# waabox/domain-mcp-server

Measured on AMD Instinct MI355X. Metric: classes indexed/sec, higher is better.
Workload: dtype n/a (CPU text indexing); 1 GPU; model=synthetic-java-spring-monorepo-2000-classes, global_batch=2000, parallelism=dp1 (one repo per rank), enrichment=none

## Files before the change

### native/srcscan/project.cpp

```cpp
#include <algorithm>
#include <chrono>
#include <dirent.h>
#include <string>
#include <unordered_map>
#include <unordered_set>

#include "srcscan.hpp"

namespace srcscan {

void go_project_files(const std::string& root, int threads, std::string& module, std::vector<FileRec>& files,
                      std::string* go_json);

namespace {

struct Entry {
    std::string name;
    bool is_dir;
};

std::vector<Entry> entries(const std::string& dir) {
    std::vector<std::pair<std::string, bool>> raw;
    std::vector<Entry> out;
    if (!list_dir(dir, raw)) return out;
// ... 46 lines not shown
    w.key("methods");
    w.begin_arr();
    for (auto& m : f.methods) {
        w.begin_obj();
        w.kv("name", m.name);
        w.kv_int("line", m.line);
        w.kv_opt("httpMethod", m.has_http_method ? &m.http_method : nullptr);
        w.kv_opt("httpPath", m.has_http_path ? &m.http_path : nullptr);
        w.str_array("exceptions", m.exceptions);
        w.end_obj();
    }
    w.end_arr();
    w.end_obj();
}

void scan_java(const std::string& root, const ScanOptions& opt, ScanResult& res) {
    std::vector<FileRec>& files = res.files;
    const std::string src_root = "src/main/java";
    std::string abs_src = join_path(root, src_root);
    if (!dir_exists(abs_src)) return;
    std::vector<std::string> rels;
    auto t = std::chrono::steady_clock::now();
    walk(abs_src, "", [](const std::string& n) { return ends_with(n, ".java"); },
         [](const std::string&) { return false; }, rels);
    res.walk_us = us_since(t);
    t = std::chrono::steady_clock::now();
    files.resize(rels.size());
    std::vector<std::string> sources(rels.size());
    parallel_for(rels.size(), opt.threads, [&](size_t k) {
        FileRec& f = files[k];
        f.rel_path = src_root + "/" + rels[k];
        f.abs_path = join_path(root, f.rel_path);
        f.identifier = dotted(strip_ext(rels[k], ".java"));
        std::string src;
        if (!read_file(f.abs_path, src)) return;
        analyze_java(src, f);
    });
    for (auto& f : files) if (!f.parsed) ++res.skipped;
    res.analyze_us = us_since(t);
    t = std::chrono::steady_clock::now();
    std::unordered_set<std::string> known;
    known.reserve(files.size() * 2);
    for (auto& f : files) known.insert(f.identifier);
    parallel_for(files.size(), opt.threads, [&](size_t k) {
        FileRec& f = files[k];
        std::unordered_set<std::string> seen;
        std::unordered_map<std::string, std::string> import_map;
        for (auto& imp : f.imports) {
            if (imp.is_asterisk) continue;
            std::string fq = imp.imported;
            if (imp.is_static) {
                size_t d = fq.rfind('.');
// ... 267 lines not shown
```

### native/srcscan/pymodule.cpp

```cpp
#include <pybind11/pybind11.h>
#include <pybind11/stl.h>
#include <sys/random.h>

#include <cctype>
#include <chrono>
#include <cstring>
#include <deque>
#include <memory>
#include <thread>
#include <unordered_map>
#include <vector>

#include "bulkwriter.hpp"
#include "gitobj.hpp"
#include "graphjson.hpp"
#include "srcscan.hpp"
#include "wire.hpp"

namespace py = pybind11;

namespace {

dbw::Batch to_batch(const std::string& sql, py::handle rows) {
    dbw::Batch b;
    b.sql = sql;
    PyObject* seq = PySequence_Fast(rows.ptr(), "rows must be a sequence");
    if (!seq) throw py::error_already_set();
    py::object keep = py::reinterpret_steal<py::object>(seq);
    const Py_ssize_t n = PySequence_Fast_GET_SIZE(seq);
    if (n == 0) return b;
    PyObject** items = PySequence_Fast_ITEMS(seq);
    PyObject* first = items[0];
    if (!PyTuple_Check(first)) throw py::type_error("rows must be tuples");
    b.ncols = static_cast<int>(PyTuple_GET_SIZE(first));
    b.values.resize(static_cast<size_t>(n) * b.ncols);
    for (Py_ssize_t r = 0; r < n; ++r) {
// ... 14 lines not shown
            } else if (PyBool_Check(o) || PyLong_Check(o)) {
                v.kind = dbw::Value::Int;
                v.i = PyLong_AsLongLong(o);
                if (v.i == -1 && PyErr_Occurred()) throw py::error_already_set();
            } else if (PyFloat_Check(o)) {
                v.kind = dbw::Value::Real;
                v.d = PyFloat_AS_DOUBLE(o);
            } else {
                throw py::type_error("unsupported column value type");
            }
        }
    }
    return b;
}

srcscan::ScanResult scan_mounted(py::list files, const std::string& language, int threads,
                                 const std::string& framework, bool go_doc = true) {
    const auto t = std::chrono::steady_clock::now();
    std::vector<py::object> hold;
    hold.reserve(files.size());
    std::vector<std::pair<std::string, std::string_view>> tree;
    tree.reserve(files.size());
    for (auto item : files) {
        auto tup = item.cast<py::tuple>();
        if (tup.size() != 2) throw py::type_error("files: (path, bytes) pairs expected");
        PyObject* content = tup[1].ptr();
        char* data = nullptr;
        Py_ssize_t n = 0;
        if (!PyBytes_Check(content) || PyBytes_AsStringAndSize(content, &data, &n) < 0)
            throw py::type_error("files: content must be bytes");
        tree.emplace_back(tup[0].cast<std::string>(), std::string_view(data, static_cast<size_t>(n)));
        hold.push_back(std::move(tup));
    }
    py::gil_scoped_release release;
    std::string root = srcscan::vfs_mount_views(tree);
    const long long mount_us =
        std::chrono::duration_cast<std::chrono::microseconds>(std::chrono::steady_clock::now() - t).count();
    srcscan::ScanOptions opt;
    opt.language = language;
    opt.threads = threads;
    opt.framework = framework;
    opt.go_doc = go_doc;
    try {
        srcscan::ScanResult r = srcscan::scan_project(root, opt);
        r.mount_us = mount_us;
        srcscan::vfs_unmount(root);
        return r;
    } catch (...) {
        srcscan::vfs_unmount(root);
        throw;
    }
}

py::str pystr(const std::string& s) {
    PyObject* o = PyUnicode_DecodeUTF8(s.data(), static_cast<Py_ssize_t>(s.size()), "replace");
    if (!o) throw py::error_already_set();
    return py::reinterpret_steal<py::str>(o);
}

void json_str_list_ascii(PyObject* seq, std::string& out) {
    static const char* hex = "0123456789abcdef";
    out.push_back('[');
    const Py_ssize_t n = PySequence_Fast_GET_SIZE(seq);
    PyObject** items = PySequence_Fast_ITEMS(seq);
    for (Py_ssize_t i = 0; i < n; ++i) {
        if (i) out.append(", ");
// ... 22 lines not shown
                        u4(c);
                    } else if (c >= 0x10000) {
                        const unsigned v = c - 0x10000;
                        u4(0xd800 | (v >> 10));
                        u4(0xdc00 | (v & 0x3ff));
                    } else {
                        out.push_back((char)c);
                    }
            }
        }
        out.push_back('"');
    }
    out.push_back(']');
}

struct RowBuilder {
    dbw::Batch b;
    explicit RowBuilder(const std::string& sql, int ncols) {
        b.sql = sql;
        b.ncols = ncols;
    }
    void null() { b.values.emplace_back(); }
    void text(const char* p, Py_ssize_t n) {
        dbw::Value v;
        v.kind = dbw::Value::Text;
        v.p = p;
        v.n = static_cast<int32_t>(n);
        b.values.push_back(v);
    }
    void str(PyObject* o) {
        if (o == Py_None) return null();
        Py_ssize_t n = 0;
        const char* p = PyUnicode_AsUTF8AndSize(o, &n);
        if (!p) throw py::error_already_set();
        text(p, n);
    }
    void owned(std::string&& s) {
        b.owned.push_back(std::move(s));
        text(b.owned.back().data(), (Py_ssize_t)b.owned.back().size());
    }
    void integer_or_null(PyObject* o) {
        if (o == Py_None) return null();
        dbw::Value v;
        v.kind = dbw::Value::Int;
        v.i = PyLong_AsLongLong(o);
        if (v.i == -1 && PyErr_Occurred()) throw py::error_already_set();
        b.values.push_back(v);
    }
    void integer(long long i) {
        dbw::Value v;
        v.kind = dbw::Value::Int;
        v.i = i;
        b.values.push_back(v);
    }
    bool empty() const { return b.values.empty(); }
};

PyObject* getattr_borrowed(PyObject* o, const char* name, std::vector<py::object>& hold) {
    PyObject* a = PyObject_GetAttrString(o, name);
    if (!a) throw py::error_already_set();
    hold.emplace_back(py::reinterpret_steal<py::object>(a));
    return a;
}

struct StrCache {
    std::unordered_map<std::string_view, PyObject*> map;
    std::deque<std::string> owned;
    ~StrCache() {
        for (auto& kv : map) Py_DECREF(kv.second);
    }
// ... 100 lines not shown
        PyTuple_SET_ITEM(rec, 0, fresh(f.rel_path));
        PyTuple_SET_ITEM(rec, 1, fresh(f.identifier));
        PyTuple_SET_ITEM(rec, 2, shared.get(f.class_type));
        PyTuple_SET_ITEM(rec, 3, PyBool_FromLong(f.entry_point));
        PyTuple_SET_ITEM(rec, 4, shared.get(f.package_name));
        PyTuple_SET_ITEM(rec, 5, shared_list(f.deps));
        PyTuple_SET_ITEM(rec, 6, params);
        PyTuple_SET_ITEM(rec, 7, methods);
        PyList_SET_ITEM(files.ptr(), k, rec);
    }
    d["files"] = files;
    d["go"] = r.go_json.empty() ? py::object(py::none()) : py::object(pystr(r.go_json));
    return d;
}

struct Uuid7Gen {
    unsigned long long ms = 0, hi = 0, lo = 0;
    Uuid7Gen() {
        unsigned char seed[10];
        if (getrandom(seed, sizeof(seed), 0) != (ssize_t)sizeof(seed)) throw std::runtime_error("getrandom failed");
        ms = (unsigned long long)std::chrono::duration_cast<std::chrono::milliseconds>(
                 std::chrono::system_clock::now().time_since_epoch())
                 .count();
        hi = ((unsigned long long)(seed[0] & 0x07) << 8) | seed[1];
        for (int j = 2; j < 10; ++j) lo = (lo << 8) | seed[j];
        lo &= 0x1FFFFFFFFFFFFFFFull;
    }
    void next(char* s) {
        static const char* hex = "0123456789abcdef";
        unsigned char b[16];
        for (int j = 0; j < 6; ++j) b[j] = (unsigned char)(ms >> (8 * (5 - j)));
        b[6] = (unsigned char)(0x70 | ((hi >> 8) & 0x0F));
        b[7] = (unsigned char)(hi & 0xFF);
        b[8] = (unsigned char)(0x80 | ((lo >> 56) & 0x3F));
        for (int j = 9; j < 16; ++j) b[j] = (unsigned char)(lo >> (8 * (15 - j)));
        if (++lo >> 62) {
            lo = 0;
            ++hi;
        }
        int k = 0;
        for (int j = 0; j < 16; ++j) {
            if (j == 4 || j == 6 || j == 8 || j == 10) s[k++] = '-';
            s[k++] = hex[b[j] >> 4];
            s[k++] = hex[b[j] & 15];
        }
    }
};

void json_ascii_list(const std::vector<std::string>& v, std::string& out) {
    static const char* hex = "0123456789abcdef";
    auto u4 = [&](unsigned c) {
        out += "\\u";
        for (int sh = 12; sh >= 0; sh -= 4) out += hex[(c >> sh) & 15];
    };
    out = "[";
    for (size_t i = 0; i < v.size(); ++i) {
        if (i) out += ", ";
        out += '"';
        const std::string& s = v[i];
        for (size_t k = 0; k < s.size();) {
            unsigned char c = (unsigned char)s[k];
            unsigned cp = c;
            size_t len = 1;
            if (c >= 0xF0 && k + 3 < s.size() + 0) { cp = ((c & 7u) << 18) | ((s[k + 1] & 63u) << 12) | ((s[k + 2] & 63u) << 6) | (s[k + 3] & 63u); len = 4; }
            else if (c >= 0xE0 && k + 2 < s.size()) { cp = ((c & 15u) << 12) | ((s[k + 1] & 63u) << 6) | (s[k + 2] & 63u); len = 3; }
            else if (c >= 0xC0 && k + 1 < s.size()) { cp = ((c & 31u) << 6) | (s[k + 1] & 63u); len = 2; }
            k += len;
            if (cp == '"') out += "\\\"";
            else if (cp == '\\') out += "\\\\";
            else if (cp == '\n') out += "\\n";
            else if (cp == '\r') out += "\\r";
            else if (cp == '\t') out += "\\t";
            else if (cp == '\b') out += "\\b";
            else if (cp == '\f') out += "\\f";
            else if (cp < 0x20 || (cp >= 0x7f && cp < 0x10000)) u4(cp);
            else if (cp >= 0x10000) {
                cp -= 0x10000;
                u4(0xD800 + (cp >> 10));
                u4(0xDC00 + (cp & 0x3FF));
            } else out += (char)cp;
        }
        out += '"';
    }
    out += "]";
}

struct StaticRowsSpec {
    dbw::BulkWriter* writer = nullptr;
    std::string pid, now, commit, cls_sql, meth_sql;
    bool commit_null = false;
};

struct StaticRowsKeep {
    std::shared_ptr<const srcscan::ScanResult> r;
    StaticRowsSpec spec;
    std::string ids;
    std::vector<size_t> first;
    std::deque<std::string> strings;
};

const std::string& normalize_class_type(const std::string& t) {
    static const std::string kTypes[] = {"CONTROLLER", "SERVICE", "REPOSITORY", "ENTITY", "DTO",
                                         "CONFIGURATION", "LISTENER", "UTILITY", "EXCEPTION", "OTHER"};
    for (const std::string& k : kTypes) {
        if (k.size() != t.size()) continue;
        bool eq = true;
        for (size_t i = 0; i < t.size() && eq; ++i) eq = std::toupper((unsigned char)t[i]) == k[i];
        if (eq) return k;
    }
    return kTypes[9];
}

void emit_static_rows(const std::shared_ptr<StaticRowsKeep>& keep) {
    const srcscan::ScanResult& r = *keep->r;
    const StaticRowsSpec& spec = keep->spec;
    std::unordered_map<std::string_view, size_t> last;
    last.reserve(r.files.size() * 2);
    size_t n_ids = 0;
    for (size_t k = 0; k < r.files.size(); ++k) last[r.files[k].identifier] = k;
    for (size_t k = 0; k < r.files.size(); ++k)
        if (last[r.files[k].identifier] == k) n_ids += 1 + r.files[k].methods.size();
    keep->ids.resize(36 * n_ids);
    keep->first.assign(r.files.size(), std::string::npos);
    Uuid7Gen gen;
    size_t at = 0;
    const int chunk = 256;
    RowBuilder cls(spec.cls_sql, 10), meth(spec.meth_sql, 10);
    int pending = 0;
    auto flush = [&]() {
        cls.b.keep = keep;
        meth.b.keep = keep;
        if (!cls.empty()) spec.writer->put(std::move(cls.b));
        if (!meth.empty()) spec.writer->put(std::move(meth.b));
        cls = RowBuilder(spec.cls_sql, 10);
        meth = RowBuilder(spec.meth_sql, 10);
        pending = 0;
    };
    auto sv = [](RowBuilder& b, const std::string& s) { b.text(s.data(), (Py_ssize_t)s.size()); };
    for (size_t k = 0; k < r.files.size(); ++k) {
        const srcscan::FileRec& f = r.files[k];
        if (last[f.identifier] != k) continue;
        if (pending == chunk) flush();
        ++pending;
        keep->first[k] = at;
        const char* cid = &keep->ids[at];
        gen.next(&keep->ids[at]);
        at += 36;
        const std::string& ident = f.identifier;
        const size_t dot = ident.rfind('.');
        cls.text(cid, 36);
        sv(cls, spec.pid);
        sv(cls, ident);
        if (dot != std::string::npos) cls.text(ident.data() + dot + 1, (Py_ssize_t)(ident.size() - dot - 1));
        else sv(cls, ident);
        if (dot != std::string::npos) cls.text(ident.data(), (Py_ssize_t)dot); else cls.null();
        sv(cls, normalize_class_type(f.class_type));
        cls.null();
        sv(cls, f.rel_path);
        sv(cls, spec.now);
        if (spec.commit_null) cls.null(); else sv(cls, spec.commit);
        for (const srcscan::MethodRec& m : f.methods) {
            gen.next(&keep->ids[at]);
            meth.text(&keep->ids[at], 36);
            at += 36;
            meth.text(cid, 36);
            sv(meth, m.name);
            meth.null();
            meth.text("[]", 2);
            if (m.exceptions.empty()) {
                meth.text("[]", 2);
            } else {
                keep->strings.emplace_back();
                json_ascii_list(m.exceptions, keep->strings.back());
                sv(meth, keep->strings.back());
            }
            if (m.has_http_method) sv(meth, m.http_method); else meth.null();
            if (m.has_http_path) sv(meth, m.http_path); else meth.null();
            meth.integer(m.line);
            sv(meth, spec.now);
        }
    }
    flush();
}

py::tuple phase1_rows(dbw::BulkWriter& writer, py::list order, py::dict units, py::object ids, py::str pid,
                      py::str now, py::handle commit_hash, const std::string& cls_sql, const std::string& meth_sql,
                      const std::string& param_sql, py::handle method_info_cls, int chunk, py::object graph_targets,
                      py::object pre_ids) {
    if (!PyType_Check(method_info_cls.ptr()) ||
        !PyType_IsSubtype((PyTypeObject*)method_info_cls.ptr(), &PyTuple_Type))
        throw py::type_error("method_info_cls must be a tuple subclass");
    auto* mi_type = (PyTypeObject*)method_info_cls.ptr();
    const bool given = !ids.is_none();
    if (given && !PyList_Check(ids.ptr())) throw py::type_error("ids must be a list or None");
    const bool pre = !pre_ids.is_none();
    if (pre && (given || !PyDict_Check(pre_ids.ptr()))) throw py::type_error("pre_ids must be a dict (and ids None)");
    const Py_ssize_t n_ids = given ? PyList_GET_SIZE(ids.ptr()) : 0;
    Py_ssize_t next_id = 0;
    py::list generated;
// ... 253 lines not shown
            if (!lst) {
                if (PyErr_Occurred()) throw py::error_already_set();
                if (PyDict_SetItem(gper, mname, lks.ptr()) < 0) throw py::error_already_set();
            } else if (PyList_SetSlice(lst, PY_SSIZE_T_MAX, PY_SSIZE_T_MAX, lks.ptr()) < 0) {
                throw py::error_already_set();
            }
        }
    }
    if (!par.empty()) writer.put(std::move(par.b));
    return py::make_tuple(n_cls, n_meth, n_par, class_ids, class_types, method_infos, methods_by_ident, links,
                          generated);
}

}

py::dict objects_and_rows(std::shared_ptr<const srcscan::ScanResult> shared, py::handle method_cls, py::object rows) {
    std::shared_ptr<StaticRowsKeep> keep;
    std::thread emitter;
    std::atomic<long long> emit_us{0};
    if (!rows.is_none() && shared->language != "go") {
        py::tuple rt = rows.cast<py::tuple>();
        if (rt.size() != 6) throw py::value_error("rows must have 6 items");
        keep = std::make_shared<StaticRowsKeep>();
        keep->r = shared;
        StaticRowsSpec& spec = keep->spec;
        spec.writer = &rt[0].cast<dbw::BulkWriter&>();
        spec.pid = rt[1].cast<std::string>();
        spec.now = rt[2].cast<std::string>();
        spec.commit_null = rt[3].is_none();
        if (!spec.commit_null) spec.commit = rt[3].cast<std::string>();
        spec.cls_sql = rt[4].cast<std::string>();
        spec.meth_sql = rt[5].cast<std::string>();
        emitter = std::thread([keep, &emit_us] {
            const auto t = std::chrono::steady_clock::now();
            emit_static_rows(keep);
            emit_us = std::chrono::duration_cast<std::chrono::microseconds>(
                          std::chrono::steady_clock::now() - t).count();
        });
    }
    py::dict d;
    try {
        const auto t = std::chrono::steady_clock::now();
        d = scan_result_objects(*shared, method_cls);
        py::dict(d["stats"])["phaseUs"].cast<py::dict>()["objects"] =
            std::chrono::duration_cast<std::chrono::microseconds>(std::chrono::steady_clock::now() - t)
                .count();
    } catch (...) {
        if (emitter.joinable()) {
            py::gil_scoped_release release;
            emitter.join();
        }
        throw;
    }
    if (emitter.joinable()) {
        {
            py::gil_scoped_release release;
            emitter.join();
        }
        py::dict(d["stats"])["phaseUs"].cast<py::dict>()["rows"] = emit_us.load();
        py::dict row_ids;
        for (size_t k = 0; k < shared->files.size(); ++k) {
            const size_t at = keep->first[k];
            if (at == std::string::npos) continue;
            const size_t nm = shared->files[k].methods.size();
            py::list mids(nm);
            for (size_t j = 0; j < nm; ++j) mids[j] = py::str(&keep->ids[at + 36 * (j + 1)], 36);
            row_ids[pystr(shared->files[k].identifier)] = py::make_tuple(py::str(&keep->ids[at], 36), mids);
        }
        d["rowIds"] = row_ids;
    }
    keep.reset();
    std::thread([](std::shared_ptr<const srcscan::ScanResult>) {}, std::move(shared)).detach();
    return d;
}

PYBIND11_MODULE(_srcscan, m) {
    m.doc() = "Native Java / TypeScript / Go source front-ends for dmcp";
    m.def(
        "scan_project",
        [](const std::string& root, const std::string& language, int threads, const std::string& framework) {
            std::string out;
            {
                py::gil_scoped_release release;
                srcscan::ScanOptions opt;
                opt.language = language;
                opt.threads = threads;
// ... 23 lines not shown
                try {
                    out = srcscan::scan_project_json(root, opt);
                } catch (...) {
                    srcscan::vfs_unmount(root);
                    throw;
                }
                srcscan::vfs_unmount(root);
            }
            return py::bytes(out);
        },
        py::arg("files"), py::arg("language") = "auto", py::arg("threads") = 0, py::arg("framework") = "");
    m.def(
        "scan_sources_objects",
        [](py::list files, const std::string& language, int threads, const std::string& framework,
           py::handle method_cls, py::object rows, bool go_doc) {
            auto r = std::make_unique<srcscan::ScanResult>(scan_mounted(files, language, threads, framework,
                                                                        go_doc));
            return objects_and_rows(std::shared_ptr<const srcscan::ScanResult>(std::move(r)), method_cls, rows);
        },
        py::arg("files"), py::arg("language"), py::arg("threads"), py::arg("framework"), py::arg("method_cls"),
        py::arg("rows") = py::none(), py::arg("go_doc") = true,
        "scan_sources as Python objects (files as tuples, methods as method_cls) -- no JSON round trip; "
        "with rows, the class / method rows are written first (ids in 'rowIds'); go_doc=False: no "
        "go-analyzer package document (Go)");
    m.def(
        "result_objects",
        [](py::bytes blob, py::handle method_cls, py::object rows) {
            auto r = std::make_unique<srcscan::ScanResult>();
            std::string err;
            bool ok;
            {
                char* data = nullptr;
                Py_ssize_t n = 0;
                if (PyBytes_AsStringAndSize(blob.ptr(), &data, &n) < 0) throw py::error_already_set();
                py::gil_scoped_release release;
                ok = srcscan::decode_result(std::string_view(data, static_cast<size_t>(n)), *r, err);
            }
            if (!ok) throw py::value_error("scan result: " + err);
            return objects_and_rows(std::shared_ptr<const srcscan::ScanResult>(std::move(r)), method_cls, rows);
        },
        py::arg("blob"), py::arg("method_cls"), py::arg("rows") = py::none(),
        "the binary ScanResult of `srcscan serve` as scan_sources_objects returns it (untrusted bytes: every "
        "length checked)");
    m.def(
        "encode_scan",
        [](py::list files, const std::string& language, int threads, const std::string& framework, bool go_doc) {
            srcscan::ScanResult r = scan_mounted(files, language, threads, framework, go_doc);
            std::string out;
            {
                py::gil_scoped_release release;
                out = srcscan::encode_result(r, true);
            }
            return py::bytes(out);
        },
// ... 198 lines not shown
        .def_property_readonly("rows_written", &dbw::BulkWriter::rows_written)
        .def("timings", [](const dbw::BulkWriter& w) {
            py::dict d;
            d["setup_ms"] = w.setup_ms();
            d["rows_ms"] = w.rows_ms();
            d["commit_ms"] = w.commit_ms();
            d["idle_ms"] = w.idle_ms();
            d["free_ms"] = w.free_ms();
            d["open_ms"] = w.open_ms();
            d["t_start_s"] = w.t_start();
            d["t_setup_s"] = w.t_setup();
            d["t_commit_s"] = w.t_commit();
            d["t_end_s"] = w.t_end();
            return d;
        });
    m.attr("ABI_VERSION") = 6;
}
```

### native/srcscan/srcscan.hpp

```cpp
#pragma once

#include <string>
#include <vector>

#include "common.hpp"

namespace srcscan {

struct MethodRec {
    std::string name;
    int line = 0;
    bool has_http_method = false, has_http_path = false;
    std::string http_method, http_path;
    std::vector<std::string> exceptions;
    std::vector<std::string> param_types;
    bool is_ctor = false;
    bool params_eligible = true;
};

struct ImportRec {
    std::string imported;
    std::string local;
    std::string source;
    bool is_static = false;
// ... 23 lines not shown
    std::string name = "unknown";
    std::string source_root = "src";
    std::vector<std::pair<std::string, std::string>> features;
};
FrameworkInfo detect_framework(std::string_view package_json);

struct GoProject;
std::string analyze_go_project_json(const std::string& root, int threads);

struct ScanOptions {
    std::string language = "auto";
    int threads = 0;
    std::string framework;
    size_t max_file_bytes = 5u * 1024u * 1024u;
    bool go_doc = true;
};

struct ScanResult {
    std::string language;
    std::string source_root = ".";
    bool has_framework = false;
    FrameworkInfo framework;
    std::string module;
    std::string go_json;
    std::vector<FileRec> files;
    int skipped = 0;
    long long elapsed_us = 0;
    long long walk_us = 0, analyze_us = 0, resolve_us = 0, mount_us = 0;
};

// ... 15 lines not shown
```

Measured before the change: 51510 classes/s.

## Stream parsed Java files to the static row emitter during the scan

Adds a PrefixSink that hands contiguous ranges of finished files to a callback while the parallel Java analysis is still running. Static row emission moves into a separate staticrows module so it can feed those ranges from a dedicated thread, overlapping row building and database writes with parsing. The aim is to hide the serial post-scan emit phase behind the scan. In exchange it adds a mutex on every file completion, needs extra bookkeeping for duplicate identifiers, and makes error propagation more involved.

```diff
diff --git a/native/srcscan/project.cpp b/native/srcscan/project.cpp
--- a/native/srcscan/project.cpp
+++ b/native/srcscan/project.cpp
@@ -1,6 +1,8 @@
 #include <algorithm>
 #include <chrono>
 #include <dirent.h>
+#include <exception>
+#include <mutex>
 #include <string>
 #include <unordered_map>
 #include <unordered_set>
@@ -84,6 +86,58 @@
     w.end_obj();
 }
 
+class PrefixSink {
+public:
+    PrefixSink(const std::vector<FileRec>& files, const ScanOptions& opt)
+        : files_(files), sink_(opt.file_sink), chunk_(std::max<size_t>(1, opt.sink_chunk)) {
+        if (sink_) done_.assign(files.size(), 0);
+    }
+
+    void done(size_t k) {
+        if (!sink_) return;
+        std::unique_lock<std::mutex> lk(mu_);
+        done_[k] = 1;
+        while (prefix_ < done_.size() && done_[prefix_]) ++prefix_;
+        deliver(lk, chunk_);
+    }
+
+    void finish() {
+        if (!sink_) return;
+        std::unique_lock<std::mutex> lk(mu_);
+        deliver(lk, 1);
+        if (error_) std::rethrow_exception(error_);
+    }
+
+private:
+    void deliver(std::unique_lock<std::mutex>& lk, size_t at_least) {
+        if (delivering_) return;
+        delivering_ = true;
+        while (!error_ && prefix_ - sent_ >= at_least) {
+            const size_t first = sent_, last = prefix_;
+            sent_ = last;
+            lk.unlock();
+            std::exception_ptr err;
+            try {
+                sink_(files_, first, last);
+            } catch (...) {
+                err = std::current_exception();
+            }
+            lk.lock();
+            if (err) error_ = err;
+        }
+        delivering_ = false;
+    }
+
+    const std::vector<FileRec>& files_;
+    const std::function<void(const std::vector<FileRec>&, size_t, size_t)>& sink_;
+    const size_t chunk_;
+    std::mutex mu_;
+    std::vector<char> done_;
+    size_t prefix_ = 0, sent_ = 0;
+    bool delivering_ = false;
+    std::exception_ptr error_;
+};
+
 void scan_java(const std::string& root, const ScanOptions& opt, ScanResult& res) {
     std::vector<FileRec>& files = res.files;
     const std::string src_root = "src/main/java";
@@ -96,16 +150,20 @@
     res.walk_us = us_since(t);
     t = std::chrono::steady_clock::now();
     files.resize(rels.size());
-    std::vector<std::string> sources(rels.size());
     parallel_for(rels.size(), opt.threads, [&](size_t k) {
         FileRec& f = files[k];
         f.rel_path = src_root + "/" + rels[k];
         f.abs_path = join_path(root, f.rel_path);
         f.identifier = dotted(strip_ext(rels[k], ".java"));
+    });
+    PrefixSink sink(files, opt);
+    parallel_for(rels.size(), opt.threads, [&](size_t k) {
+        FileRec& f = files[k];
         std::string src;
-        if (!read_file(f.abs_path, src)) return;
-        analyze_java(src, f);
+        if (read_file(f.abs_path, src)) analyze_java(src, f);
+        sink.done(k);
     });
+    sink.finish();
     for (auto& f : files) if (!f.parsed) ++res.skipped;
     res.analyze_us = us_since(t);
     t = std::chrono::steady_clock::now();
diff --git a/native/srcscan/pymodule.cpp b/native/srcscan/pymodule.cpp
--- a/native/srcscan/pymodule.cpp
+++ b/native/srcscan/pymodule.cpp
@@ -15,11 +15,18 @@
 #include "gitobj.hpp"
 #include "graphjson.hpp"
 #include "srcscan.hpp"
+#include "staticrows.hpp"
 #include "wire.hpp"
 
 namespace py = pybind11;
 
 namespace {
+
+using staticrows::StaticRowsEmitter;
+using staticrows::StaticRowsKeep;
+using staticrows::StaticRowsSpec;
+using staticrows::stream_rows_enabled;
+using staticrows::Uuid7Gen;
 
 dbw::Batch to_batch(const std::string& sql, py::handle rows) {
     dbw::Batch b;
@@ -64,8 +71,10 @@
     return b;
 }
 
-srcscan::ScanResult scan_mounted(py::list files, const std::string& language, int threads,
-                                 const std::string& framework, bool go_doc = true) {
+void scan_mounted_into(py::list files, const std::string& language, int threads, const std::string& framework,
+                       bool go_doc, srcscan::ScanResult& r,
+                       std::function<void(const std::vector<srcscan::FileRec>&, size_t, size_t)> sink = nullptr,
+                       const std::function<void()>& after_scan = nullptr) {
     const auto t = std::chrono::steady_clock::now();
     std::vector<py::object> hold;
     hold.reserve(files.size());
@@ -91,15 +100,23 @@
     opt.threads = threads;
     opt.framework = framework;
     opt.go_doc = go_doc;
+    opt.file_sink = std::move(sink);
     try {
-        srcscan::ScanResult r = srcscan::scan_project(root, opt);
+        srcscan::scan_project_into(root, opt, r);
         r.mount_us = mount_us;
-        srcscan::vfs_unmount(root);
-        return r;
+        if (after_scan) after_scan();
     } catch (...) {
         srcscan::vfs_unmount(root);
         throw;
     }
+    srcscan::vfs_unmount(root);
+}
+
+srcscan::ScanResult scan_mounted(py::list files, const std::string& language, int threads,
+                                 const std::string& framework, bool go_doc = true) {
+    srcscan::ScanResult r;
+    scan_mounted_into(files, language, threads, framework, go_doc, r);
+    return r;
 }
 
 py::str pystr(const std::string& s) {
@@ -152,30 +169,14 @@
     out.push_back(']');
 }
 
-struct RowBuilder {
-    dbw::Batch b;
-    explicit RowBuilder(const std::string& sql, int ncols) {
-        b.sql = sql;
-        b.ncols = ncols;
-    }
-    void null() { b.values.emplace_back(); }
-    void text(const char* p, Py_ssize_t n) {
-        dbw::Value v;
-        v.kind = dbw::Value::Text;
-        v.p = p;
-        v.n = static_cast<int32_t>(n);
-        b.values.push_back(v);
-    }
+struct RowBuilder : staticrows::TextRows {
+    using staticrows::TextRows::TextRows;
     void str(PyObject* o) {
         if (o == Py_None) return null();
         Py_ssize_t n = 0;
         const char* p = PyUnicode_AsUTF8AndSize(o, &n);
         if (!p) throw py::error_already_set();
-        text(p, n);
-    }
-    void owned(std::string&& s) {
-        b.owned.push_back(std::move(s));
-        text(b.owned.back().data(), (Py_ssize_t)b.owned.back().size());
+        text(p, static_cast<size_t>(n));
     }
     void integer_or_null(PyObject* o) {
         if (o == Py_None) return null();
@@ -185,13 +186,6 @@
         if (v.i == -1 && PyErr_Occurred()) throw py::error_already_set();
         b.values.push_back(v);
     }
-    void integer(long long i) {
-        dbw::Value v;
-        v.kind = dbw::Value::Int;
-        v.i = i;
-        b.values.push_back(v);
-    }
-    bool empty() const { return b.values.empty(); }
 };
 
 PyObject* getattr_borrowed(PyObject* o, const char* name, std::vector<py::object>& hold) {
@@ -322,175 +316,6 @@
     return d;
 }
 
-struct Uuid7Gen {
-    unsigned long long ms = 0, hi = 0, lo = 0;
-    Uuid7Gen() {
-        unsigned char seed[10];
-        if (getrandom(seed, sizeof(seed), 0) != (ssize_t)sizeof(seed)) throw std::runtime_error("getrandom failed");
-        ms = (unsigned long long)std::chrono::duration_cast<std::chrono::milliseconds>(
-                 std::chrono::system_clock::now().time_since_epoch())
-                 .count();
-        hi = ((unsigned long long)(seed[0] & 0x07) << 8) | seed[1];
-        for (int j = 2; j < 10; ++j) lo = (lo << 8) | seed[j];
-        lo &= 0x1FFFFFFFFFFFFFFFull;
-    }
-    void next(char* s) {
-        static const char* hex = "0123456789abcdef";
-        unsigned char b[16];
-        for (int j = 0; j < 6; ++j) b[j] = (unsigned char)(ms >> (8 * (5 - j)));
-        b[6] = (unsigned char)(0x70 | ((hi >> 8) & 0x0F));
-        b[7] = (unsigned char)(hi & 0xFF);
-        b[8] = (unsigned char)(0x80 | ((lo >> 56) & 0x3F));
-        for (int j = 9; j < 16; ++j) b[j] = (unsigned char)(lo >> (8 * (15 - j)));
-        if (++lo >> 62) {
-            lo = 0;
-            ++hi;
-        }
-        int k = 0;
-        for (int j = 0; j < 16; ++j) {
-            if (j == 4 || j == 6 || j == 8 || j == 10) s[k++] = '-';
-            s[k++] = hex[b[j] >> 4];
-            s[k++] = hex[b[j] & 15];
-        }
-    }
-};
-
-void json_ascii_list(const std::vector<std::string>& v, std::string& out) {
-    static const char* hex = "0123456789abcdef";
-    auto u4 = [&](unsigned c) {
-        out += "\\u";
-        for (int sh = 12; sh >= 0; sh -= 4) out += hex[(c >> sh) & 15];
-    };
-    out = "[";
-    for (size_t i = 0; i < v.size(); ++i) {
-        if (i) out += ", ";
-        out += '"';
-        const std::string& s = v[i];
-        for (size_t k = 0; k < s.size();) {
-            unsigned char c = (unsigned char)s[k];
-            unsigned cp = c;
-            size_t len = 1;
-            if (c >= 0xF0 && k + 3 < s.size() + 0) { cp = ((c & 7u) << 18) | ((s[k + 1] & 63u) << 12) | ((s[k + 2] & 63u) << 6) | (s[k + 3] & 63u); len = 4; }
-            else if (c >= 0xE0 && k + 2 < s.size()) { cp = ((c & 15u) << 12) | ((s[k + 1] & 63u) << 6) | (s[k + 2] & 63u); len = 3; }
-            else if (c >= 0xC0 && k + 1 < s.size()) { cp = ((c & 31u) << 6) | (s[k + 1] & 63u); len = 2; }
-            k += len;
-            if (cp == '"') out += "\\\"";
-            else if (cp == '\\') out += "\\\\";
-            else if (cp == '\n') out += "\\n";
-            else if (cp == '\r') out += "\\r";
-            else if (cp == '\t') out += "\\t";
-            else if (cp == '\b') out += "\\b";
-            else if (cp == '\f') out += "\\f";
-            else if (cp < 0x20 || (cp >= 0x7f && cp < 0x10000)) u4(cp);
-            else if (cp >= 0x10000) {
-                cp -= 0x10000;
-                u4(0xD800 + (cp >> 10));
-                u4(0xDC00 + (cp & 0x3FF));
-            } else out += (char)cp;
-        }
-        out += '"';
-    }
-    out += "]";
-}
-
-struct StaticRowsSpec {
-    dbw::BulkWriter* writer = nullptr;
-    std::string pid, now, commit, cls_sql, meth_sql;
-    bool commit_null = false;
-};
-
-struct StaticRowsKeep {
-    std::shared_ptr<const srcscan::ScanResult> r;
-    StaticRowsSpec spec;
-    std::string ids;
-    std::vector<size_t> first;
-    std::deque<std::string> strings;
-};
-
-const std::string& normalize_class_type(const std::string& t) {
-    static const std::string kTypes[] = {"CONTROLLER", "SERVICE", "REPOSITORY", "ENTITY", "DTO",
-                                         "CONFIGURATION", "LISTENER", "UTILITY", "EXCEPTION", "OTHER"};
-    for (const std::string& k : kTypes) {
-        if (k.size() != t.size()) continue;
-        bool eq = true;
-        for (size_t i = 0; i < t.size() && eq; ++i) eq = std::toupper((unsigned char)t[i]) == k[i];
-        if (eq) return k;
-    }
-    return kTypes[9];
-}
-
-void emit_static_rows(const std::shared_ptr<StaticRowsKeep>& keep) {
-    const srcscan::ScanResult& r = *keep->r;
-    const StaticRowsSpec& spec = keep->spec;
-    std::unordered_map<std::string_view, size_t> last;
-    last.reserve(r.files.size() * 2);
-    size_t n_ids = 0;
-    for (size_t k = 0; k < r.files.size(); ++k) last[r.files[k].identifier] = k;
-    for (size_t k = 0; k < r.files.size(); ++k)
-        if (last[r.files[k].identifier] == k) n_ids += 1 + r.files[k].methods.size();
-    keep->ids.resize(36 * n_ids);
-    keep->first.assign(r.files.size(), std::string::npos);
-    Uuid7Gen gen;
-    size_t at = 0;
-    const int chunk = 256;
-    RowBuilder cls(spec.cls_sql, 10), meth(spec.meth_sql, 10);
-    int pending = 0;
-    auto flush = [&]() {
-        cls.b.keep = keep;
-        meth.b.keep = keep;
-        if (!cls.empty()) spec.writer->put(std::move(cls.b));
-        if (!meth.empty()) spec.writer->put(std::move(meth.b));
-        cls = RowBuilder(spec.cls_sql, 10);
-        meth = RowBuilder(spec.meth_sql, 10);
-        pending = 0;
-    };
-    auto sv = [](RowBuilder& b, const std::string& s) { b.text(s.data(), (Py_ssize_t)s.size()); };
-    for (size_t k = 0; k < r.files.size(); ++k) {
-        const srcscan::FileRec& f = r.files[k];
-        if (last[f.identifier] != k) continue;
-        if (pending == chunk) flush();
-        ++pending;
-        keep->first[k] = at;
-        const char* cid = &keep->ids[at];
-        gen.next(&keep->ids[at]);
-        at += 36;
-        const std::string& ident = f.identifier;
-        const size_t dot = ident.rfind('.');
-        cls.text(cid, 36);
-        sv(cls, spec.pid);
-        sv(cls, ident);
-        if (dot != std::string::npos) cls.text(ident.data() + dot + 1, (Py_ssize_t)(ident.size() - dot - 1));
-        else sv(cls, ident);
-        if (dot != std::string::npos) cls.text(ident.data(), (Py_ssize_t)dot); else cls.null();
-        sv(cls, normalize_class_type(f.class_type));
-        cls.null();
-        sv(cls, f.rel_path);
-        sv(cls, spec.now);
-        if (spec.commit_null) cls.null(); else sv(cls, spec.commit);
-        for (const srcscan::MethodRec& m : f.methods) {
-            gen.next(&keep->ids[at]);
-            meth.text(&keep->ids[at], 36);
-            at += 36;
-            meth.text(cid, 36);
-            sv(meth, m.name);
-            meth.null();
-            meth.text("[]", 2);
-            if (m.exceptions.empty()) {
-                meth.text("[]", 2);
-            } else {
-                keep->strings.emplace_back();
-                json_ascii_list(m.exceptions, keep->strings.back());
-                sv(meth, keep->strings.back());
-            }
-            if (m.has_http_method) sv(meth, m.http_method); else meth.null();
-            if (m.has_http_path) sv(meth, m.http_path); else meth.null();
-            meth.integer(m.line);
-            sv(meth, spec.now);
-        }
-    }
-    flush();
-}
-
 py::tuple phase1_rows(dbw::BulkWriter& writer, py::list order, py::dict units, py::object ids, py::str pid,
                       py::str now, py::handle commit_hash, const std::string& cls_sql, const std::string& meth_sql,
                       const std::string& param_sql, py::handle method_info_cls, int chunk, py::object graph_targets,
@@ -774,28 +599,36 @@
 
 }
 
-py::dict objects_and_rows(std::shared_ptr<const srcscan::ScanResult> shared, py::handle method_cls, py::object rows) {
-    std::shared_ptr<StaticRowsKeep> keep;
+std::unique_ptr<StaticRowsEmitter> rows_emitter(py::object rows, std::shared_ptr<const srcscan::ScanResult> shared) {
+    if (rows.is_none()) return nullptr;
+    py::tuple rt = rows.cast<py::tuple>();
+    if (rt.size() != 6) throw py::value_error("rows must have 6 items");
+    auto keep = std::make_shared<StaticRowsKeep>();
+    keep->r = std::move(shared);
+    StaticRowsSpec& spec = keep->spec;
+    spec.writer = &rt[0].cast<dbw::BulkWriter&>();
+    spec.pid = rt[1].cast<std::string>();
+    spec.now = rt[2].cast<std::string>();
+    spec.commit_null = rt[3].is_none();
+    if (!spec.commit_null) spec.commit = rt[3].cast<std::string>();
+    spec.cls_sql = rt[4].cast<std::string>();
+    spec.meth_sql = rt[5].cast<std::string>();
+    return std::make_unique<StaticRowsEmitter>(std::move(keep));
+}
+
+py::dict objects_and_rows(std::shared_ptr<const srcscan::ScanResult> shared, py::handle method_cls,
+                          std::unique_ptr<StaticRowsEmitter> em) {
+    if (em && shared->language == "go") em.reset();
     std::thread emitter;
-    std::atomic<long long> emit_us{0};
-    if (!rows.is_none() && shared->language != "go") {
-        py::tuple rt = rows.cast<py::tuple>();
-        if (rt.size() != 6) throw py::value_error("rows must have 6 items");
-        keep = std::make_shared<StaticRowsKeep>();
-        keep->r = shared;
-        StaticRowsSpec& spec = keep->spec;
-        spec.writer = &rt[0].cast<dbw::BulkWriter&>();
-        spec.pid = rt[1].cast<std::string>();
-        spec.now = rt[2].cast<std::string>();
-        spec.commit_null = rt[3].is_none();
-        if (!spec.commit_null) spec.commit = rt[3].cast<std::string>();
-        spec.cls_sql = rt[4].cast<std::string>();
-        spec.meth_sql = rt[5].cast<std::string>();
-        emitter = std::thread([keep, &emit_us] {
-            const auto t = std::chrono::steady_clock::now();
-            emit_static_rows(keep);
-            emit_us = std::chrono::duration_cast<std::chrono::microseconds>(
-                          std::chrono::steady_clock::now() - t).count();
+    std::exception_ptr emit_error;
+    if (em && !em->finished()) {
+        emitter = std::thread([&em, &shared, &emit_error] {
+            try {
+                em->feed(shared->files, em->fed(), shared->files.size());
+                em->finish();
+            } catch (...) {
+                emit_error = std::current_exception();
+            }
         });
     }
     py::dict d;
@@ -812,24 +645,28 @@
         }
         throw;
     }
-    if (emitter.joinable()) {
-        {
+    if (em) {
+        if (emitter.joinable()) {
             py::gil_scoped_release release;
             emitter.join();
         }
-        py::dict(d["stats"])["phaseUs"].cast<py::dict>()["rows"] = emit_us.load();
+        if (emit_error) std::rethrow_exception(emit_error);
+        const StaticRowsKeep& keep = *em->keep();
+        py::dict stats(d["stats"]);
+        stats["phaseUs"].cast<py::dict>()["rows"] = em->us();
+        stats["streamedFiles"] = em->streamed;
         py::dict row_ids;
-        for (size_t k = 0; k < shared->files.size(); ++k) {
-            const size_t at = keep->first[k];
-            if (at == std::string::npos) continue;
+        for (size_t k = 0; k < keep.first.size(); ++k) {
+            const char* at = keep.first[k];
+            if (at == nullptr) continue;
             const size_t nm = shared->files[k].methods.size();
             py::list mids(nm);
-            for (size_t j = 0; j < nm; ++j) mids[j] = py::str(&keep->ids[at + 36 * (j + 1)], 36);
-            row_ids[pystr(shared->files[k].identifier)] = py::make_tuple(py::str(&keep->ids[at], 36), mids);
+            for (size_t j = 0; j < nm; ++j) mids[j] = py::str(at + 36 * (j + 1), 36);
+            row_ids[pystr(shared->files[k].identifier)] = py::make_tuple(py::str(at, 36), mids);
         }
         d["rowIds"] = row_ids;
     }
-    keep.reset();
+    em.reset();
     std::thread([](std::shared_ptr<const srcscan::ScanResult>) {}, std::move(shared)).detach();
     return d;
 }
@@ -883,9 +720,18 @@
         "scan_sources_objects",
         [](py::list files, const std::string& language, int threads, const std::string& framework,
            py::handle method_cls, py::object rows, bool go_doc) {
-            auto r = std::make_unique<srcscan::ScanResult>(scan_mounted(files, language, threads, framework,
-                                                                        go_doc));
-            return objects_and_rows(std::shared_ptr<const srcscan::ScanResult>(std::move(r)), method_cls, rows);
+            auto r = std::make_shared<srcscan::ScanResult>();
+            std::unique_ptr<StaticRowsEmitter> em = rows_emitter(rows, r);
+            if (em && stream_rows_enabled()) {
+                staticrows::EmitterThread feeder(*em);
+                scan_mounted_into(
+                    files, language, threads, framework, go_doc, *r,
+                    [&feeder](const std::vector<srcscan::FileRec>&, size_t a, size_t b) { feeder.push(a, b); },
+                    [&feeder] { feeder.close(); });
+            } else {
+                scan_mounted_into(files, language, threads, framework, go_doc, *r);
+            }
+            return objects_and_rows(std::move(r), method_cls, std::move(em));
         },
         py::arg("files"), py::arg("language"), py::arg("threads"), py::arg("framework"), py::arg("method_cls"),
         py::arg("rows") = py::none(), py::arg("go_doc") = true,
@@ -906,7 +752,8 @@
                 ok = srcscan::decode_result(std::string_view(data, static_cast<size_t>(n)), *r, err);
             }
             if (!ok) throw py::value_error("scan result: " + err);
-            return objects_and_rows(std::shared_ptr<const srcscan::ScanResult>(std::move(r)), method_cls, rows);
+            std::shared_ptr<const srcscan::ScanResult> shared(std::move(r));
+            return objects_and_rows(shared, method_cls, rows_emitter(rows, shared));
         },
         py::arg("blob"), py::arg("method_cls"), py::arg("rows") = py::none(),
         "the binary ScanResult of `srcscan serve` as scan_sources_objects returns it (untrusted bytes: every "
@@ -1135,5 +982,5 @@
             d["t_end_s"] = w.t_end();
             return d;
         });
-    m.attr("ABI_VERSION") = 6;
-}
+    m.attr("ABI_VERSION") = 7;
+}
diff --git a/native/srcscan/srcscan.hpp b/native/srcscan/srcscan.hpp
--- a/native/srcscan/srcscan.hpp
+++ b/native/srcscan/srcscan.hpp
@@ -1,5 +1,6 @@
 #pragma once
 
+#include <functional>
 #include <string>
 #include <vector>
 
@@ -61,6 +62,8 @@
     std::string framework;
     size_t max_file_bytes = 5u * 1024u * 1024u;
     bool go_doc = true;
+    std::function<void(const std::vector<FileRec>& files, size_t first, size_t last)> file_sink;
+    size_t sink_chunk = 64;
 };
 
 struct ScanResult {
diff --git a/native/srcscan/staticrows.hpp b/native/srcscan/staticrows.hpp
--- /dev/null
+++ b/native/srcscan/staticrows.hpp
@@ -0,0 +1,348 @@
+#pragma once
+
+#include <sys/random.h>
+
+#include <algorithm>
+#include <cctype>
+#include <chrono>
+#include <condition_variable>
+#include <cstdlib>
+#include <deque>
+#include <exception>
+#include <memory>
+#include <mutex>
+#include <stdexcept>
+#include <thread>
+#include <utility>
+#include <string>
+#include <string_view>
+#include <unordered_map>
+#include <vector>
+
+#include "bulkwriter.hpp"
+#include "srcscan.hpp"
+
+namespace staticrows {
+
+struct TextRows {
+    dbw::Batch b;
+    explicit TextRows(const std::string& sql, int ncols) {
+        b.sql = sql;
+        b.ncols = ncols;
+    }
+    void null() { b.values.emplace_back(); }
+    void text(const char* p, size_t n) {
+        dbw::Value v;
+        v.kind = dbw::Value::Text;
+        v.p = p;
+        v.n = static_cast<int32_t>(n);
+        b.values.push_back(v);
+    }
+    void owned(std::string&& s) {
+        b.owned.push_back(std::move(s));
+        text(b.owned.back().data(), b.owned.back().size());
+    }
+    void integer(long long i) {
+        dbw::Value v;
+        v.kind = dbw::Value::Int;
+        v.i = i;
+        b.values.push_back(v);
+    }
+    bool empty() const { return b.values.empty(); }
+};
+
+struct Uuid7Gen {
+    unsigned long long ms = 0, hi = 0, lo = 0;
+    Uuid7Gen() {
+        unsigned char seed[10];
+        if (getrandom(seed, sizeof(seed), 0) != (ssize_t)sizeof(seed)) throw std::runtime_error("getrandom failed");
+        ms = (unsigned long long)std::chrono::duration_cast<std::chrono::milliseconds>(
+                 std::chrono::system_clock::now().time_since_epoch())
+                 .count();
+        hi = ((unsigned long long)(seed[0] & 0x07) << 8) | seed[1];
+        for (int j = 2; j < 10; ++j) lo = (lo << 8) | seed[j];
+        lo &= 0x1FFFFFFFFFFFFFFFull;
+    }
+    void next(char* s) {
+        static const char* hex = "0123456789abcdef";
+        unsigned char b[16];
+        for (int j = 0; j < 6; ++j) b[j] = (unsigned char)(ms >> (8 * (5 - j)));
+        b[6] = (unsigned char)(0x70 | ((hi >> 8) & 0x0F));
+        b[7] = (unsigned char)(hi & 0xFF);
+        b[8] = (unsigned char)(0x80 | ((lo >> 56) & 0x3F));
+        for (int j = 9; j < 16; ++j) b[j] = (unsigned char)(lo >> (8 * (15 - j)));
+        if (++lo >> 62) {
+            lo = 0;
+            ++hi;
+        }
+        int k = 0;
+        for (int j = 0; j < 16; ++j) {
+            if (j == 4 || j == 6 || j == 8 || j == 10) s[k++] = '-';
+            s[k++] = hex[b[j] >> 4];
+            s[k++] = hex[b[j] & 15];
+        }
+    }
+};
+
+inline void json_ascii_list(const std::vector<std::string>& v, std::string& out) {
+    static const char* hex = "0123456789abcdef";
+    auto u4 = [&](unsigned c) {
+        out += "\\u";
+        for (int sh = 12; sh >= 0; sh -= 4) out += hex[(c >> sh) & 15];
+    };
+    out = "[";
+    for (size_t i = 0; i < v.size(); ++i) {
+        if (i) out += ", ";
+        out += '"';
+        const std::string& s = v[i];
+        for (size_t k = 0; k < s.size();) {
+            unsigned char c = (unsigned char)s[k];
+            unsigned cp = c;
+            size_t len = 1;
+            if (c >= 0xF0 && k + 3 < s.size() + 0) { cp = ((c & 7u) << 18) | ((s[k + 1] & 63u) << 12) | ((s[k + 2] & 63u) << 6) | (s[k + 3] & 63u); len = 4; }
+            else if (c >= 0xE0 && k + 2 < s.size()) { cp = ((c & 15u) << 12) | ((s[k + 1] & 63u) << 6) | (s[k + 2] & 63u); len = 3; }
+            else if (c >= 0xC0 && k + 1 < s.size()) { cp = ((c & 31u) << 6) | (s[k + 1] & 63u); len = 2; }
+            k += len;
+            if (cp == '"') out += "\\\"";
+            else if (cp == '\\') out += "\\\\";
+            else if (cp == '\n') out += "\\n";
+            else if (cp == '\r') out += "\\r";
+            else if (cp == '\t') out += "\\t";
+            else if (cp == '\b') out += "\\b";
+            else if (cp == '\f') out += "\\f";
+            else if (cp < 0x20 || (cp >= 0x7f && cp < 0x10000)) u4(cp);
+            else if (cp >= 0x10000) {
+                cp -= 0x10000;
+                u4(0xD800 + (cp >> 10));
+                u4(0xDC00 + (cp & 0x3FF));
+            } else out += (char)cp;
+        }
+        out += '"';
+    }
+    out += "]";
+}
+
+struct StaticRowsSpec {
+    dbw::BulkWriter* writer = nullptr;
+    std::string pid, now, commit, cls_sql, meth_sql;
+    bool commit_null = false;
+};
+
+struct StaticRowsKeep {
+    std::shared_ptr<const srcscan::ScanResult> r;
+    StaticRowsSpec spec;
+    std::vector<std::unique_ptr<char[]>> id_blocks;
+    std::vector<const char*> first;
+    std::deque<std::string> strings;
+};
+
+inline const std::string& normalize_class_type(const std::string& t) {
+    static const std::string kTypes[] = {"CONTROLLER", "SERVICE", "REPOSITORY", "ENTITY", "DTO",
+                                         "CONFIGURATION", "LISTENER", "UTILITY", "EXCEPTION", "OTHER"};
+    for (const std::string& k : kTypes) {
+        if (k.size() != t.size()) continue;
+        bool eq = true;
+        for (size_t i = 0; i < t.size() && eq; ++i) eq = std::toupper((unsigned char)t[i]) == k[i];
+        if (eq) return k;
+    }
+    return kTypes[9];
+}
+
+class StaticRowsEmitter {
+public:
+    explicit StaticRowsEmitter(std::shared_ptr<StaticRowsKeep> keep)
+        : keep_(std::move(keep)), cls_(keep_->spec.cls_sql, 10), meth_(keep_->spec.meth_sql, 10) {}
+
+    const std::shared_ptr<StaticRowsKeep>& keep() const { return keep_; }
+    size_t fed() const { return next_; }
+    size_t streamed = 0;
+    bool finished() const { return finished_; }
+    long long us() const { return us_; }
+
+    void feed(const std::vector<srcscan::FileRec>& files, size_t a, size_t b) {
+        const auto t = std::chrono::steady_clock::now();
+        if (&files != &keep_->r->files || a != next_ || b > files.size() || finished_)
+            throw std::logic_error("static rows: ranges must cover the scan's files in order");
+        if (!started_) {
+            started_ = true;
+            last_.reserve(files.size() * 2);
+            for (size_t k = 0; k < files.size(); ++k) last_[files[k].identifier] = k;
+            keep_->first.assign(files.size(), nullptr);
+        }
+        for (size_t k = a; k < b; ++k) emit(files[k], k);
+        next_ = b;
+        us_ += since(t);
+    }
+
+    void finish() {
+        const auto t = std::chrono::steady_clock::now();
+        flush(false);
+        finished_ = true;
+        us_ += since(t);
+    }
+
+private:
+    static constexpr int kChunk = 256;
+    static constexpr size_t kIdBlock = 36 * 4096;
+
+    static long long since(std::chrono::steady_clock::time_point t) {
+        return std::chrono::duration_cast<std::chrono::microseconds>(std::chrono::steady_clock::now() - t).count();
+    }
+
+    char* ids_for(size_t n) {
+        const size_t need = 36 * n;
+        if (need > block_left_) {
+            block_left_ = std::max(need, kIdBlock);
+            keep_->id_blocks.emplace_back(new char[block_left_]);
+            block_at_ = keep_->id_blocks.back().get();
+        }
+        char* p = block_at_;
+        block_at_ += need;
+        block_left_ -= need;
+        return p;
+    }
+
+    void flush(bool more) {
+        const StaticRowsSpec& spec = keep_->spec;
+        cls_.b.keep = keep_;
+        meth_.b.keep = keep_;
+        const size_t n_meth = meth_.b.values.size();
+        if (!cls_.empty()) spec.writer->put(std::move(cls_.b));
+        if (!meth_.empty()) spec.writer->put(std::move(meth_.b));
+        cls_ = TextRows(spec.cls_sql, 10);
+        meth_ = TextRows(spec.meth_sql, 10);
+        if (more && n_meth) {
+            cls_.b.values.reserve(static_cast<size_t>(kChunk) * 10);
+            meth_.b.values.reserve(n_meth + n_meth / 4);
+        }
+        pending_ = 0;
+    }
+
+    static void sv(TextRows& b, const std::string& s) { b.text(s.data(), s.size()); }
+
+    void emit(const srcscan::FileRec& f, size_t k) {
+        const StaticRowsSpec& spec = keep_->spec;
+        if (last_[f.identifier] != k) return;
+        if (pending_ == kChunk) flush(true);
+        ++pending_;
+        char* at = ids_for(1 + f.methods.size());
+        keep_->first[k] = at;
+        const char* cid = at;
+        gen_.next(at);
+        at += 36;
+        const std::string& ident = f.identifier;
+        const size_t dot = ident.rfind('.');
+        TextRows& cls = cls_;
+        TextRows& meth = meth_;
+        cls.text(cid, 36);
+        sv(cls, spec.pid);
+        sv(cls, ident);
+        if (dot != std::string::npos) cls.text(ident.data() + dot + 1, (ident.size() - dot - 1));
+        else sv(cls, ident);
+        if (dot != std::string::npos) cls.text(ident.data(), dot); else cls.null();
+        sv(cls, normalize_class_type(f.class_type));
+        cls.null();
+        sv(cls, f.rel_path);
+        sv(cls, spec.now);
+        if (spec.commit_null) cls.null(); else sv(cls, spec.commit);
+        for (const srcscan::MethodRec& m : f.methods) {
+            gen_.next(at);
+            meth.text(at, 36);
+            at += 36;
+            meth.text(cid, 36);
+            sv(meth, m.name);
+            meth.null();
+            meth.text("[]", 2);
+            if (m.exceptions.empty()) {
+                meth.text("[]", 2);
+            } else {
+                keep_->strings.emplace_back();
+                json_ascii_list(m.exceptions, keep_->strings.back());
+                sv(meth, keep_->strings.back());
+            }
+            if (m.has_http_method) sv(meth, m.http_method); else meth.null();
+            if (m.has_http_path) sv(meth, m.http_path); else meth.null();
+            meth.integer(m.line);
+            sv(meth, spec.now);
+        }
+    }
+
+    std::shared_ptr<StaticRowsKeep> keep_;
+    std::unordered_map<std::string_view, size_t> last_;
+    Uuid7Gen gen_;
+    TextRows cls_, meth_;
+    int pending_ = 0;
+    size_t next_ = 0;
+    char* block_at_ = nullptr;
+    size_t block_left_ = 0;
+    bool started_ = false, finished_ = false;
+    long long us_ = 0;
+};
+
+class EmitterThread {
+public:
+    explicit EmitterThread(StaticRowsEmitter& em) : em_(em), thread_([this] { run(); }) {}
+    ~EmitterThread() { stop(); }
+    EmitterThread(const EmitterThread&) = delete;
+    EmitterThread& operator=(const EmitterThread&) = delete;
+
+    void push(size_t a, size_t b) {
+        {
+            std::lock_guard<std::mutex> g(mu_);
+            ranges_.emplace_back(a, b);
+        }
+        cv_.notify_one();
+    }
+
+    void close() {
+        stop();
+        if (error_) std::rethrow_exception(error_);
+    }
+
+private:
+    void stop() noexcept {
+        if (!thread_.joinable()) return;
+        {
+            std::lock_guard<std::mutex> g(mu_);
+            closed_ = true;
+        }
+        cv_.notify_one();
+        thread_.join();
+    }
+
+    void run() noexcept {
+        const std::vector<srcscan::FileRec>& files = em_.keep()->r->files;
+        try {
+            for (;;) {
+                std::pair<size_t, size_t> r;
+                {
+                    std::unique_lock<std::mutex> lk(mu_);
+                    cv_.wait(lk, [this] { return closed_ || !ranges_.empty(); });
+                    if (ranges_.empty()) break;
+                    r = ranges_.front();
+                    ranges_.pop_front();
+                }
+                em_.feed(files, r.first, r.second);
+                em_.streamed += r.second - r.first;
+            }
+            if (em_.fed() == files.size()) em_.finish();
+        } catch (...) {
+            error_ = std::current_exception();
+        }
+    }
+
+    StaticRowsEmitter& em_;
+    std::mutex mu_;
+    std::condition_variable cv_;
+    std::deque<std::pair<size_t, size_t>> ranges_;
+    bool closed_ = false;
+    std::exception_ptr error_;
+    std::thread thread_;
+};
+
+inline bool stream_rows_enabled() {
+    const char* e = std::getenv("DMCP_STREAM_ROWS");
+    return e == nullptr || e[0] != '0';
+}
+
+}
diff --git a/native/srcscan/stream_rows_check.cpp b/native/srcscan/stream_rows_check.cpp
--- /dev/null
+++ b/native/srcscan/stream_rows_check.cpp
@@ -0,0 +1,193 @@
+#include <unistd.h>
+
+#include <atomic>
+#include <cstdio>
+#include <cstdlib>
+#include <memory>
+#include <string>
+#include <vector>
+
+#include "bulkwriter.hpp"
+#include "sqlite_min.hpp"
+#include "srcscan.hpp"
+#include "staticrows.hpp"
+
+namespace {
+
+constexpr int OPEN_CREATE = 0x00000004;
+
+const char* kSchema =
+    "CREATE TABLE source_classes (id TEXT PRIMARY KEY, project_id TEXT NOT NULL, full_class_name TEXT NOT NULL,"
+    " simple_name TEXT NOT NULL, package_name TEXT, class_type TEXT NOT NULL, description TEXT, source_file TEXT,"
+    " created_at TEXT NOT NULL, commit_hash TEXT, UNIQUE(project_id, full_class_name));"
+    "CREATE TABLE source_methods (id TEXT PRIMARY KEY, class_id TEXT NOT NULL, method_name TEXT NOT NULL,"
+    " description TEXT, business_logic TEXT, exceptions TEXT, http_method TEXT, http_path TEXT,"
+    " line_number INTEGER, created_at TEXT NOT NULL);"
+    "CREATE INDEX idx_methods_class ON source_methods(class_id);";
+const char* kClassSql = "INSERT INTO source_classes VALUES (?, ?, ?, ?, ?, ?, ?, ?, ?, ?)";
+const char* kMethodSql = "INSERT INTO source_methods VALUES (?, ?, ?, ?, ?, ?, ?, ?, ?, ?)";
+
+int failures = 0;
+void check(bool ok, const char* what) {
+    if (!ok) {
+        std::fprintf(stderr, "FAILED: %s\n", what);
+        ++failures;
+    }
+}
+
+struct Db {
+    sqlite3* db = nullptr;
+    explicit Db(const std::string& path, int flags) {
+        if (sqlite3_open_v2(path.c_str(), &db, flags, nullptr) != sqlite_min::OK) {
+            std::fprintf(stderr, "cannot open %s\n", path.c_str());
+            std::exit(2);
+        }
+    }
+    ~Db() { sqlite3_close_v2(db); }
+    void exec(const char* sql) {
+        if (sqlite3_exec(db, sql, nullptr, nullptr, nullptr) != sqlite_min::OK) {
+            std::fprintf(stderr, "%s: %s\n", sql, sqlite3_errmsg(db));
+            std::exit(2);
+        }
+    }
+    long long scalar(const char* sql) {
+        long long v = -1;
+        auto cb = [](void* out, int, char** cols, char**) {
+            *static_cast<long long*>(out) = cols[0] ? std::atoll(cols[0]) : 0;
+            return 0;
+        };
+        if (sqlite3_exec(db, sql, cb, &v, nullptr) != sqlite_min::OK) {
+            std::fprintf(stderr, "%s: %s\n", sql, sqlite3_errmsg(db));
+            std::exit(2);
+        }
+        return v;
+    }
+};
+
+std::vector<std::pair<std::string, std::string>> java_tree(int n, long long& methods, long long& classes) {
+    std::vector<std::pair<std::string, std::string>> tree;
+    methods = 0;
+    for (int k = 0; k < n; ++k) {
+        const std::string name = "C" + std::to_string(k);
+        std::string src = "package co.check.p" + std::to_string(k % 7) + ";\n\n";
+        if (k % 3 == 0) src += "@org.springframework.web.bind.annotation.RestController\n";
+        src += "public class " + name + " {\n";
+        const int nm = k % 5;
+        for (int j = 0; j < nm; ++j) {
+            if (k % 3 == 0) src += "    @GetMapping(\"/c" + std::to_string(k) + "/m" + std::to_string(j) + "\")\n";
+            src += "    public void m" + std::to_string(j) + "(String a)" +
+                   (j % 2 ? " throws java.io.IOException, IllegalStateException" : "") + " {\n    }\n\n";
+        }
+        src += "}\n";
+        methods += nm;
+        tree.emplace_back("src/main/java/co/check/p" + std::to_string(k % 7) + "/" + name + ".java", std::move(src));
+    }
+    classes = n;
+    if (n > 0) {
+        tree.emplace_back("src/main/java/x/y/Twin.java", "package x.y;\npublic class Twin { void a() {} void b() {} }\n");
+        tree.emplace_back("src/main/java/x.y/Twin.java", "package x.y;\npublic class Twin { void c() {} }\n");
+        classes += 1;
+        methods += 1;
+    }
+    tree.emplace_back("src/main/java/co/check/Broken.java", std::string("\xff\xfe{{{(\"\0class", 12));
+    classes += 1;
+    return tree;
+}
+
+size_t scan_streaming(const std::vector<std::pair<std::string, std::string>>& tree, int threads,
+                      dbw::BulkWriter& writer, size_t sink_chunk) {
+    auto result = std::make_shared<srcscan::ScanResult>();
+    auto keep = std::make_shared<staticrows::StaticRowsKeep>();
+    keep->r = result;
+    keep->spec.writer = &writer;
+    keep->spec.pid = "project-1";
+    keep->spec.now = "2024-01-01T00:00:00.000Z";
+    keep->spec.commit_null = true;
+    keep->spec.cls_sql = kClassSql;
+    keep->spec.meth_sql = kMethodSql;
+    staticrows::StaticRowsEmitter em(keep);
+    keep.reset();
+    staticrows::EmitterThread feeder(em);
+    std::atomic<int> in_sink{0};
+    srcscan::ScanOptions opt;
+    opt.language = "java";
+    opt.threads = threads;
+    opt.sink_chunk = sink_chunk;
+    size_t expect_first = 0;
+    opt.file_sink = [&](const std::vector<srcscan::FileRec>& files, size_t a, size_t b) {
+        check(in_sink.fetch_add(1) == 0, "sink calls never overlap");
+        check(a == expect_first && a < b && b <= files.size(), "ranges are contiguous and increasing");
+        expect_first = b;
+        feeder.push(a, b);
+        in_sink.fetch_sub(1);
+    };
+    auto copy = tree;
+    const std::string root = srcscan::vfs_mount(std::move(copy));
+    srcscan::scan_project_into(root, opt, *result);
+    srcscan::vfs_unmount(root);
+    check(expect_first == result->files.size(), "every file went through the sink before the scan returned");
+    feeder.close();
+    check(em.fed() == result->files.size() && em.finished(), "the emitter thread emitted every file");
+    return em.streamed;
+}
+
+}
+
+int main(int argc, char** argv) {
+    const int n = argc > 1 ? std::atoi(argv[1]) : 700;
+    const int threads = argc > 2 ? std::atoi(argv[2]) : 8;
+    char path[] = "/tmp/stream_rows_check_XXXXXX";
+    const int fd = mkstemp(path);
+    if (fd < 0) return 2;
+    close(fd);
+    {
+        Db db(path, sqlite_min::OPEN_READWRITE | OPEN_CREATE);
+        db.exec(kSchema);
+    }
+    long long methods = 0, classes = 0;
+    const auto tree = java_tree(n, methods, classes);
+    {
+        dbw::BulkWriter writer(path, 5000, {});
+        const size_t streamed = scan_streaming(tree, threads, writer, 64);
+        check(streamed == tree.size(), "all files streamed");
+        writer.commit();
+        const std::string err = writer.wait();
+        check(err.empty(), "commit succeeded");
+        check(writer.rows_written() == classes + methods, "rows written == classes + methods");
+    }
+    {
+        Db db(path, sqlite_min::OPEN_READWRITE);
+        check(db.scalar("SELECT COUNT(*) FROM source_classes") == classes, "class rows");
+        check(db.scalar("SELECT COUNT(*) FROM source_methods") == methods, "method rows");
+        check(db.scalar("SELECT COUNT(*) FROM source_methods m WHERE NOT EXISTS "
+                        "(SELECT 1 FROM source_classes c WHERE c.id = m.class_id)") == 0, "methods point at classes");
+        check(db.scalar("SELECT COUNT(*) FROM (SELECT id, LAG(id) OVER (ORDER BY rowid) AS prev FROM source_classes) "
+                        "WHERE prev IS NOT NULL AND prev >= id") == 0, "class ids ascend in file order");
+        if (n > 0) {
+            check(db.scalar("SELECT COUNT(*) FROM source_classes WHERE full_class_name = 'x.y.Twin' "
+                            "AND source_file = 'src/main/java/x.y/Twin.java'") == 1, "the later twin wins");
+            check(db.scalar("SELECT COUNT(*) FROM source_methods m JOIN source_classes c ON c.id = m.class_id "
+                            "WHERE c.full_class_name = 'x.y.Twin'") == 1, "the later twin's methods only");
+        }
+    }
+    {
+        dbw::BulkWriter writer(path, 5000, {});
+        for (const char* sql : {"DELETE FROM source_methods", "DELETE FROM source_classes"}) {
+            dbw::Batch del;
+            del.sql = sql;
+            writer.put(std::move(del));
+        }
+        scan_streaming(tree, threads, writer, 1);
+        writer.abort();
+        check(writer.wait() == "aborted", "abort reported");
+    }
+    {
+        Db db(path, sqlite_min::OPEN_READWRITE);
+        check(db.scalar("SELECT COUNT(*) FROM source_classes") == classes, "class rows after the rollback");
+        check(db.scalar("SELECT COUNT(*) FROM source_methods") == methods, "method rows after the rollback");
+    }
+    unlink(path);
+    std::printf("%s: %d files, %lld classes, %lld methods, %d threads\n", failures ? "FAILED" : "ok",
+                (int)tree.size(), classes, methods, threads);
+    return failures ? 1 : 0;
+}
```

Result: faster. 60360 classes/s (median of 6 runs) (+17.2%).
